# iliasam/STM32F4_SDR_GPS

Measured on AMD Instinct MI355X. Metric: acquisition hypotheses/sec (PRN x Doppler x phase), higher is better.
Workload: dtype u1 (MX-FP4 operands, exact f32 accumulation)

## Files before the change

### stm32f4_sdr_gps_amd/csrc/gpsx_mx_transposed.hpp

```cpp
#pragma once
#include <stdint.h>

constexpr int kGpsxMxtLocals = 64;
constexpr int kGpsxMxtKeyShift = 6;
constexpr int kGpsxKeyShift = 11;

constexpr int gpsx_mxt_q0_tile(int wave) { return 8 * (wave >> 1) + (wave & 1); }
constexpr int gpsx_mxt_row(int h, int r) { return (r & 3) + 8 * (r >> 2) + 4 * h; }
constexpr int gpsx_mxt_q(int wave, int h, int j, int r) { return 32 * (gpsx_mxt_q0_tile(wave) + 2 * j) + gpsx_mxt_row(h, r); }
constexpr int gpsx_mxt_local(int j, int r) { return 16 * j + r; }
constexpr uint32_t gpsx_mxt_code(int j, int r) { return (uint32_t)(kGpsxMxtLocals - 1 - gpsx_mxt_local(j, r)); }
constexpr uint32_t gpsx_mxt_local_key(uint32_t bits, int j, int r) { return (bits << kGpsxMxtKeyShift) | gpsx_mxt_code(j, r); }
constexpr int gpsx_mxt_q_of_local(int q_first, int local)
{
  return q_first + ((local & 48) << 2) + ((local & 12) << 1) + (local & 3);
}
constexpr uint32_t gpsx_mxt_global_key(uint32_t local_key, int q_first, int half)
{
  const int local = (int)((local_key & (kGpsxMxtLocals - 1)) ^ (kGpsxMxtLocals - 1));
  const int q = gpsx_mxt_q_of_local(q_first, local);
  return ((local_key >> kGpsxMxtKeyShift) << kGpsxKeyShift) | (uint32_t)(2047 - (2 * q + half));
}
constexpr int gpsx_mxt_group(int lane) { return (lane & 31) >> 3; }
```

### stm32f4_sdr_gps_amd/csrc/k_acq_mx.hip

```cpp
#include "gpsx_mx_parts.hpp"
#include "gpsx_mx_transposed.hpp"

namespace gpsx {

__global__ void k_build_mx_tables(const u32 *__restrict__ chipbits, int n_slots, u32 *__restrict__ mx_a, u32 *__restrict__ mx_t)
{
  const int n_sets = (n_slots + 31) / 32;
  const int idx = blockIdx.x * blockDim.x + threadIdx.x;
  const int per_set = 16 * 2 * 32 * 4 + 1032;
  if (idx >= n_sets * per_set)
    return;
  const int set = idx / per_set, r = idx - set * per_set;
  if (r < 16 * 2 * 32 * 4) {
    const int dw = r & 3, p = (r >> 2) & 31, h = (r >> 7) & 1, kappa = r >> 8;
    const int slot = 32 * set + p;
    const u32 word = slot < n_slots ? chipbits[(size_t)slot * 32 + 2 * kappa + h] : 0u;
    mx_a[(size_t)set * (16 * 2 * 32 * 4) + r] = spread8((word >> (8 * dw)) & 0xFFu) << 1;
  } else {
    const int c = r - 16 * 2 * 32 * 4 - 1;
    u32 w = 0;
    if (c >= 0 && c < kChips)
      for (int p = 0; p < 32; p++) {
        const int slot = 32 * set + p;
        if (slot < n_slots)
          w |= ((chipbits[(size_t)slot * 32 + (c >> 5)] >> (c & 31)) & 1u) << p;
      }
    mx_t[(size_t)set * 1032 + (c + 1)] = w;
  }
}

void launch_build_mx_tables(hipStream_t s, const uint32_t *d_chipbits, int n_slots, uint32_t *d_mx_a, uint32_t *d_mx_t)
{
  const int n_sets = (n_slots + 31) / 32;
  const int n = n_sets * (16 * 2 * 32 * 4 + 1032);
  hipLaunchKernelGGL(k_build_mx_tables, dim3((n + 255) / 256), dim3(256), 0, s, d_chipbits, n_slots, d_mx_a, d_mx_t);
}

namespace {

constexpr int kMxNoSet = -1;
constexpr int kPasses = 17;
constexpr int kPassesAnchor = 16;
constexpr int kAnchorDwords = 392;

__device__ __forceinline__ void mx_planes_half(MxSharedCore &sh, int t0_lo, int v, int lane)
{
  const int iq = v >> 1, t0_first = t0_lo + 4 * (v & 1);
  const int t0 = t0_first + (lane & 3), rot = lane >> 2;
#pragma unroll 1
  for (int it = 0; it < 2; it++) {
    const int w = rot + 16 * it;
    const u32 *src = &sh.d[iq][16 * w];
    u32 bits = 0;
#pragma unroll
    for (int k = 0; k < 16; k++) {
      const int kk = (k + rot) & 15;
      const u32 sk = src[kk];
      bits |= ((sk >> t0) & 1u) << (2 * kk);
      bits |= ((sk >> (16 + t0)) & 1u) << (2 * kk + 1);
    }
    sh.plane[iq][t0][w] = bits;
  }
  __builtin_amdgcn_fence(__ATOMIC_ACQ_REL, "wavefront");
  asm volatile("s_waitcnt lgkmcnt(0)" ::: "memory");
#pragma unroll 1
  for (int m = lane; m < 4 * (kPlaneWordsMx - 32); m += 64) {
    const int r = m / (kPlaneWordsMx - 32), w = 32 + m % (kPlaneWordsMx - 32);
    u32 *pl = sh.plane[iq][t0_first + r];
    pl[w] = mx_plane_ext_word(pl, w);
  }
}

__device__ __forceinline__ void mx_anchor_build(MxSharedCore &sh, u32 *dst, int tid)
{
  const int iq = tid >> 8, j = tid & 255;
  const u32 *dd = sh.d[iq];
  u64 bits = 0;
#pragma unroll
  for (int e = 0; e < 8; e++) {
    const int pos = 16 * wrap1023(8 * j + e);
    const u32 sum = pop16(__builtin_amdgcn_alignbit(dd[(pos >> 5) + 1], dd[pos >> 5], (u32)(pos & 31)));
    bits |= (u64)gpsx_anchor_code((int)sum) << (6 * e);
  }
  const u32 lo = (u32)bits, hi = (u32)(bits >> 32);
  const u32 lo_pair = dpp<0xB1>(lo, lo);
  u32 *d3 = dst + iq * kAnchorDwords + 3 * (j >> 1);
  if (j & 1) {
    d3[2] = (lo >> 16) | (hi << 16);
  } else {
    d3[0] = lo;
    d3[1] = hi | (lo_pair << 16);
  }
}

struct AnchorRaw {
  u32 d[7];
};
__device__ __forceinline__ AnchorRaw mx_anchor_raw(lds_cu32 *w, int dw)
{
  AnchorRaw r;
#pragma unroll
  for (int i = 0; i < 7; i++)
    r.d[i] = w[dw + i];
  return r;
}
__device__ __forceinline__ v8i mx_anchor_frag(const AnchorRaw &r, u32 shift)
{
  v8i f = {0, 0, 0, 0, 0, 0, 0, 0};
#pragma unroll
  for (int i = 0; i < 6; i++)
    f[i] = (int)__builtin_amdgcn_alignbit(r.d[i + 1], r.d[i], shift);
  return f;
}
template <int S, int NT>
__device__ __forceinline__ void mx_anchor_step(lds_cu32 *wi, lds_cu32 *wq, const v4i *ca, v4i (&a)[16], v8i &fi, v8i &fq,
                                               v16f (&acc)[2][NT], u32 shift)
{
  constexpr int kSteps = 16 + NT - 1;
  constexpr bool more = S + 1 < kSteps;
  AnchorRaw ri, rq;
  if constexpr (more) {
    ri = mx_anchor_raw(wi, 12 * (S + 1));
    rq = mx_anchor_raw(wq, 12 * (S + 1));
    if constexpr (S + 1 < 16)
      a[S + 1] = ca[(S + 1) * 64];
  }
  constexpr int j_lo = S - 15 > 0 ? S - 15 : 0, j_hi = S < NT - 1 ? S : NT - 1;
#pragma unroll
  for (int j = j_lo; j <= j_hi; j++) {
    acc[0][j] = __builtin_amdgcn_mfma_scale_f32_32x32x64_f8f6f4(fi, widen(a[S - j]), acc[0][j], 3, 4, 0, kScaleTwo, 0, kScaleA);
    acc[1][j] = __builtin_amdgcn_mfma_scale_f32_32x32x64_f8f6f4(fq, widen(a[S - j]), acc[1][j], 3, 4, 0, kScaleTwo, 0, kScaleA);
  }
  if constexpr (more) {
    __builtin_amdgcn_sched_group_barrier(0x100, S + 1 < 16 ? 9 : 8, 0);
    __builtin_amdgcn_sched_group_barrier(0x008, 2 * (j_hi - j_lo + 1), 0);
  }
  __builtin_amdgcn_sched_barrier(0);
  if constexpr (more) {
    fi = mx_anchor_frag(ri, shift);
    fq = mx_anchor_frag(rq, shift);
    __builtin_amdgcn_sched_barrier(0);
    mx_anchor_step<S + 1, NT>(wi, wq, ca, a, fi, fq, acc, shift);
  }
}
template <int NT>
__device__ __forceinline__ void mx_anchor_pass(const MxSharedCore &sh, const u32 *anchor, int lane, int q0_tile, v16f (&acc)[2][NT])
{
  const int n = lane & 31, h = lane >> 5;
  const u32 shift = (u32)(6 * n) & 31u;
  lds_cu32 *wi = lds_opaque(anchor + 6 * (q0_tile + h) + ((6 * n) >> 5));
  lds_cu32 *wq = lds_opaque(anchor + kAnchorDwords + 6 * (q0_tile + h) + ((6 * n) >> 5));
  const v4i *ca = &sh.chips_a[0][h][n];
  v4i a[16];
  v8i fi = mx_anchor_frag(mx_anchor_raw(wi, 0), shift), fq = mx_anchor_frag(mx_anchor_raw(wq, 0), shift);
  a[0] = ca[0];
  mx_anchor_step<0, NT>(wi, wq, ca, a, fi, fq, acc, shift);
}

__device__ __forceinline__ void mx_vector_build_direct(MxShared &sh, int which, int t0s, u32 *e8_dst, int tid)
{
  const int iq = tid >> 8, j = tid & 255;
  const u32 *dd = sh.d[iq];
  u32 w2[2] = {0, 0};
#pragma unroll
  for (int e = 0; e < 16; e++) {
    const int k = wrap1023(8 * j + e);
    const int pos = 16 * k + t0s;
    const u32 sum = pop16(__builtin_amdgcn_alignbit(dd[(pos >> 5) + 1], dd[pos >> 5], (u32)(pos & 31)));
    const u32 code = which == 0 ? (0xFEC0u >> (4u * (sum & 3u))) & 0xFu : (0xEDCA0u >> (4u * (sum >> 2))) & 0xFu;
    w2[e >> 3] |= code << (4 * (e & 7));
  }
  u32 *dst = e8_dst + (iq * 8) * kCopyDwords + j;
#pragma unroll
  for (int c = 0; c < 8; c++)
    dst[c * kCopyDwords] = c ? __builtin_amdgcn_alignbit(w2[1], w2[0], 4u * (u32)c) : w2[0];
}

__device__ __forceinline__ void mx_direct_terms(const MxShared &sh, int lane, int q0_tile, v16f (&acc)[2][kMxTiles], int t0s,
                                                int win_start, int win_stop)
{
  const int n = lane & 31, h = lane >> 5;
  const int b = t0s & 7, half = t0s >> 3;
  const u32 low = (1u << b) - 1u, high = (0xFFFFu << b) & 0xFFFFu;
  const float fh = (float)half;
  const u32 f22 = sh.chip_t[1022 + 1] >> (4 * h), f21 = sh.chip_t[1021 + 1] >> (4 * h);
  float popw[2], beta[2];
#pragma unroll
  for (int s = 0; s < 2; s++) {
    const int pw = (int)__popc(sh.d[s][0] & 0xFFu);
    popw[s] = (float)pw;
    beta[s] = (float)(16 - b - 2 * pw);
  }
#pragma unroll
  for (int j = 0; j < kMxTiles; j++) {
    const int q = 32 * (q0_tile + 2 * j) + n;
    const bool exists = q < kChips;
    const int qc = exists ? q : 0;
    const int o = 2 * qc + half;
    const float tq = (qc > 0) ? fh : 0.0f;
    float k0[2], k21[2], k22[2], kb[2];
#pragma unroll
    for (int s = 0; s < 2; s++) {
      const int fa = 2 * (int)__popc(lds_byte(sh.d[s], o) & low) - b;
      int fp = 0, gl = 0, gh = 0;
      if (qc > 0 || half == 0) {
        const int o2 = o >= 2 ? o : 2;
        const u32 prev = lds_byte(sh.d[s], o2 - 2) | (lds_byte(sh.d[s], o2 - 1) << 8);
        fp = (int)__popc(prev);
        gl = b - 2 * (int)__popc(prev & low);
        gh = 16 - b - 2 * (int)__popc(prev & high);
      }
      k0[s] = -(fh * popw[s] + tq * (float)fp) * kAccScale;
      k21[s] = -tq * (float)gl * kAccScale;
      k22[s] = ((float)fa - tq * (float)gh) * kAccScale;
      kb[s] = -fh * beta[s] * kAccScale;
    }
    const float ka = -fh * (float)b * kAccScale;
    if (half) {
      const bool in0 = exists && 2 * q >= win_start && 2 * q < win_stop;
      const bool in1 = exists && 2 * q + 1 >= win_start && 2 * q + 1 < win_stop;
      if (in0 != in1) {
        k0[0] += in1 ? -kOutside : kOutside;
        k0[1] += in1 ? -kOutside : kOutside;
      }
    }
    const u32 w1 = sh.chip_t[(exists ? kChips - 1 - q : 0) + 1] >> (4 * h);
    const u32 w0 = sh.chip_t[(exists ? kChips - 2 - q : -1) + 1] >> (4 * h);
#pragma unroll
    for (int r = 0; r < 16; r++) {
      const int pb = (r & 3) + 8 * (r >> 2);
      const float c22 = (float)((f22 >> pb) & 1u), c21 = (float)((f21 >> pb) & 1u);
      const float ca = (float)((w0 >> pb) & 1u), cb = (float)((w1 >> pb) & 1u);
      acc[0][j][r] += k0[0] + ca * ka + cb * kb[0] + c21 * k21[0] + c22 * k22[0];
      acc[1][j][r] += k0[1] + ca * ka + cb * kb[1] + c21 * k21[1] + c22 * k22[1];
    }
  }
}

template <bool S16>
struct SumRecT {
  u32 w[S16 ? 2 : 3];
};
template <bool S16>
__device__ __forceinline__ void sums_unpack(const SumRecT<S16> &r, u32 (&s)[4])
{
  if constexpr (S16) {
    s[0] = r.w[0] & 0xFFFFu;
    s[1] = r.w[0] >> 16;
    s[2] = r.w[1] & 0xFFFFu;
    s[3] = r.w[1] >> 16;
  } else {
    s[0] = r.w[0] & 0xFFFFFFu;
    s[1] = __builtin_amdgcn_alignbit(r.w[1], r.w[0], 24u) & 0xFFFFFFu;
    s[2] = __builtin_amdgcn_alignbit(r.w[2], r.w[1], 16u) & 0xFFFFFFu;
    s[3] = r.w[2] >> 8;
  }
}
template <bool S16>
__device__ __forceinline__ SumRecT<S16> sums_pack(const u32 (&s)[4])
{
  SumRecT<S16> r;
  if constexpr (S16) {
    r.w[0] = __builtin_amdgcn_perm(s[1], s[0], 0x05040100u);
    r.w[1] = __builtin_amdgcn_perm(s[3], s[2], 0x05040100u);
  } else {
    r.w[0] = s[0] | (s[1] << 24);
    r.w[1] = (s[1] >> 8) | (s[2] << 16);
    r.w[2] = (s[2] >> 16) | (s[3] << 8);
  }
  return r;
}

typedef unsigned short us2 __attribute__((ext_vector_type(2)));
__device__ __forceinline__ u32 pk_add_sat_u16(u32 a, u32 b)
{
  return __builtin_bit_cast(u32, __builtin_elementwise_add_sat(__builtin_bit_cast(us2, a), __builtin_bit_cast(us2, b)));
}

template <bool S16>
struct alignas(8) RecPairT {
  SumRecT<S16> a, b;
};
template <int FIRST, int COUNT, bool S16>
__device__ __forceinline__ void mx_prefetch_sums(const u32 *__restrict__ energy, const u32 *__restrict__ zero_recs, int lane,
                                                 int t0, bool ms_first, SumRecT<S16> (&pre)[16])
{
  static_assert(FIRST % 2 == 0 && COUNT % 2 == 0, "records move in pairs");
  if constexpr (S16) {
    const SumRecT<S16> *e2 = ms_first ? reinterpret_cast<const SumRecT<S16> *>(zero_recs) + (size_t)lane * 2
                                      : reinterpret_cast<const SumRecT<S16> *>(energy) + (size_t)(t0 * kMxTiles) * 256 + (size_t)lane * 2;
#pragma unroll
    for (int i = FIRST; i < FIRST + COUNT; i += 2) {
      const RecPairT<S16> rp = *reinterpret_cast<const RecPairT<S16> *>(&e2[(size_t)(i >> 2) * 256 + (size_t)((i & 3) >> 1) * 128]);
      pre[i] = rp.a;
      pre[i + 1] = rp.b;
    }
    return;
  }
  const SumRecT<S16> *e4 = ms_first ? reinterpret_cast<const SumRecT<S16> *>(zero_recs) + (size_t)lane * 4
                                    : reinterpret_cast<const SumRecT<S16> *>(energy) + ((size_t)(t0 * kMxTiles) * 64 + lane) * 4;
#pragma unroll
  for (int i = FIRST; i < FIRST + COUNT; i += 2) {
    const RecPairT<S16> rp = *reinterpret_cast<const RecPairT<S16> *>(&e4[(size_t)(i >> 2) * 256 + (i & 3)]);
    pre[i] = rp.a;
    pre[i + 1] = rp.b;
  }
}

template <bool MULTI, bool SEARCH, bool S16>
__device__ __forceinline__ void mx_epilogue(MxShared &sh, int lane, int q0_tile, int t0, const v16f (&acc)[2][kMxTiles],
                                            u32 group_mask, u32 *__restrict__ energy, const u32 *__restrict__ zero_recs,
                                            SumRecT<S16> (&pre)[MULTI ? 16 : 1], bool ms_first, u32 &witness)
{
  typedef SumRecT<S16> SumRec;
  constexpr bool ms_last = SEARCH;
  const int n = lane & 31, h = lane >> 5;
  const int b = t0 & 7, half = t0 >> 3;
  constexpr bool DIRECT = MULTI;
  u32 *slot = SEARCH ? &sh.part[b][4 * h][0][n] : nullptr;
  u32 best[SEARCH && !DIRECT ? 16 : 1], total[SEARCH && !DIRECT ? 16 : 1];
#pragma unroll
  for (int r = 0; r < (SEARCH && !DIRECT ? 16 : 1); r++) {
    best[r] = 0;
    total[r] = 0;
  }
  SumRec *e4 = reinterpret_cast<SumRec *>(energy) + ((size_t)(t0 * kMxTiles) * 64 + lane) * 4;
  mx_round_toward_zero();
#pragma unroll
  for (int j = 0; j < kMxTiles; j++) {
    const int q = 32 * (q0_tile + 2 * j) + n;
    const u32 key_lo = (u32)(2047 - (2 * q + half));
    if constexpr (MULTI) {
      if (j == 0)
        mx_prefetch_sums<8, 8, S16>(energy, zero_recs, lane, t0, ms_first, pre);
    }
    constexpr int GS = MULTI ? 4 : 8;
    SumRec held{};
#pragma unroll
    for (int r0 = 0; r0 < 16; r0 += GS) {
      u32 prev[GS];
#pragma unroll
      for (int i = 0; i < GS; i++)
        prev[i] = 0;
      if (MULTI && !(S16 && !SEARCH)) {
#pragma unroll
        for (int g = 0; g < GS / 4; g++) {
          u32 p4[4];
          sums_unpack<S16>(pre[MULTI ? j * 4 + r0 / 4 + g : 0], p4);
#pragma unroll
          for (int i = 0; i < 4; i++) {
            prev[4 * g + i] = p4[i];
            if constexpr (S16)
              witness = max(witness, p4[i]);
          }
        }
      }
      SumRec *e_rec = e4 + (size_t)j * 256 + r0 / 4;
      u32 out[GS];
      float ev[GS];
      u32 e_max = 0;
#pragma unroll
      for (int i = 0; i < GS; i++) {
        ev[i] = clip_square_sum(acc[0][j][r0 + i], acc[1][j][r0 + i]);
        e_max = max(e_max, __float_as_uint(ev[i]));
      }
      const bool small = __builtin_amdgcn_ballot_w64(e_max >= 0x3C800000u ) == 0;
      u32 mag[GS];
      constexpr bool PACKED = MULTI && S16 && !SEARCH;
      if (small) {
#pragma unroll
        for (int i = 0; i < GS; i++)
          mag[i] = PACKED ? root_bits_small(ev[i]) : (u32)(int)(__builtin_amdgcn_sqrtf(ev[i]) * kRootGuard);
      } else {
        float ci[GS], cq[GS];
#pragma unroll
        for (int i = 0; i < GS; i++) {
          ci[i] = acc[0][j][r0 + i];
          cq[i] = acc[1][j][r0 + i];
        }
        mx_roots_exact<GS>(ci, cq, mag);
      }
      if constexpr (PACKED) {
        const SumRec &pr = pre[j * 4 + r0 / 4];
        SumRec nr;
        nr.w[0] = pk_add_sat_u16(pr.w[0], __builtin_amdgcn_perm(mag[1], mag[0], 0x05040100u));
        nr.w[1] = pk_add_sat_u16(pr.w[1], __builtin_amdgcn_perm(mag[3], mag[2], 0x05040100u));
        if ((r0 / 4) & 1) {
          RecPairT<S16> both;
          both.a = held;
          both.b = nr;
          SumRec *e_pair = reinterpret_cast<SumRec *>(energy) + (size_t)(t0 * kMxTiles + j) * 256 + (size_t)(r0 / 8) * 128 + (size_t)lane * 2;
          *reinterpret_cast<RecPairT<S16> *>(e_pair) = both;
        } else {
          held = nr;
        }
        __builtin_amdgcn_sched_barrier(0);
        continue;
      }
#pragma unroll
      for (int i = 0; i < GS; i++) {
        const int r = r0 + i;
        u32 val = mag[i];
        if (MULTI)
          val += prev[i];
        out[i] = val;
        if (SEARCH && DIRECT) {
          const int p_off = ((r & 3) + 8 * (r >> 2)) * 64;
          atomicMax(slot + p_off, (val << 11) | key_lo);
          atomicAdd(slot + p_off + 32, val);
        } else if (SEARCH) {
          const u32 key = (val << 11) | key_lo;
          best[DIRECT ? 0 : r] = key > best[DIRECT ? 0 : r] ? key : best[DIRECT ? 0 : r];
          total[DIRECT ? 0 : r] += val;
        }
      }
      if (MULTI && !ms_last) {
#pragma unroll
        for (int g = 0; g < GS / 4; g++) {
          const u32 o4[4] = {out[4 * g], out[4 * g + 1], out[4 * g + 2], out[4 * g + 3]};
          e_rec[g] = sums_pack<S16>(o4);
        }
      }
      if (SEARCH && !DIRECT) {
#pragma unroll
        for (int i = 0; i < GS; i++)
          asm volatile("" : "+v"(best[DIRECT ? 0 : r0 + i]), "+v"(total[DIRECT ? 0 : r0 + i]));
      }
      __builtin_amdgcn_sched_barrier(0);
    }
  }
  mx_round_to_nearest();
  if (SEARCH && !DIRECT) {
#pragma unroll
    for (int r = 0; r < 16; r++) {
      const int p_off = ((r & 3) + 8 * (r >> 2)) * 64;
      atomicMax(slot + p_off, best[DIRECT ? 0 : r]);
      atomicAdd(slot + p_off + 32, total[DIRECT ? 0 : r]);
    }
  }
}

__device__ __forceinline__ void mx_epilogue_store(int lane, int q0_tile, int t0, const v16f (&acc)[2][kMxTiles], u32 group_mask,
                                                  uint16_t *__restrict__ plane0, size_t prn_stride, int slot0, int n_prn)
{
  const int n = lane & 31, h = lane >> 5;
#pragma unroll
  for (int j = 0; j < kMxTiles; j++) {
    const int q = 32 * (q0_tile + 2 * j) + n;
    uint16_t *v = plane0 + (size_t)t0 * 1024 + (size_t)(q & 3) * 256 + (size_t)(q >> 2);
#pragma unroll
    for (int g = 0; g < 4; g++) {
#pragma unroll
      for (int rr = 0; rr < 4; rr++) {
        const int r = 4 * g + rr;
        const int p = (r & 3) + 8 * (r >> 2) + 4 * h;
        const u32 val = mag8_f32(acc[0][j][r], acc[1][j][r]);
        if (((group_mask >> g) & 1u) && slot0 + p < n_prn)
          v[(size_t)p * prn_stride] = (uint16_t)val;
      }
      __builtin_amdgcn_sched_barrier(0);
    }
  }
}

constexpr int kHsStride = 1026;
struct MxSingleShared {
  MxSharedCore mx;
  MxFold fold;
  alignas(16) u32 part[8][2][2][32];
  alignas(16) float2 hs[2][kHsStride];
};

struct MxtWindow {
  int lo0, hi0, lo1, hi1;
};
__device__ __forceinline__ MxtWindow mxt_window(int win_start, int win_stop)
{
  MxtWindow w;
  w.lo0 = (win_start + 1) >> 1;
  w.hi0 = min(kChips, (win_stop + 1) >> 1);
  w.lo1 = win_start >> 1;
  w.hi1 = min(kChips, win_stop >> 1);
  return w;
}
__device__ __forceinline__ bool mxt_wave_whole(int q0_tile, int win_start, int win_stop)
{
  const MxtWindow w = mxt_window(win_start, win_stop);
  const int q_lo = 32 * q0_tile, q_hi = 32 * (q0_tile + 2 * (kMxTiles - 1)) + 31;
  return q_lo >= w.lo0 && q_hi < w.hi1;
}

__device__ __forceinline__ void mxt_init_acc(const u32 *ones, int lane, int q0_tile, v16f (&acc)[2][kMxTiles], int win_start,
                                             int win_stop, int pass_bias)
{
  const float base_i = (float)((int)ones[0] + 8192 - kHalf - pass_bias) * kAccScale,
              base_q = (float)((int)ones[1] + 8192 - kHalf - pass_bias) * kAccScale;
  if (mxt_wave_whole(q0_tile, win_start, win_stop)) {
#pragma unroll
    for (int j = 0; j < kMxTiles; j++)
#pragma unroll
      for (int r = 0; r < 16; r++) {
        acc[0][j][r] = base_i;
        acc[1][j][r] = base_q;
      }
  } else {
    const MxtWindow w = mxt_window(win_start, win_stop);
    const int h = lane >> 5;
    const u32 span = (u32)max(w.hi0 - w.lo0, 0);
#pragma unroll
    for (int j = 0; j < kMxTiles; j++)
#pragma unroll
      for (int r = 0; r < 16; r++) {
        const int q = 32 * (q0_tile + 2 * j) + gpsx_mxt_row(h, r);
        const bool in_win = (u32)(q - w.lo0) < span;
        acc[0][j][r] = in_win ? base_i : base_i + kOutside;
        acc[1][j][r] = in_win ? base_q : base_q + kOutside;
      }
  }
}

__device__ __forceinline__ void mxt_half_switch_build(const MxSharedCore &sh, float2 (*hs)[kHsStride], int t, int n)
{
  const int popw[2] = {(int)__popc(sh.d[0][0] & 0xFFu), (int)__popc(sh.d[1][0] & 0xFFu)};
#pragma unroll 1
  for (int m = t; m < 512; m += n) {
    float row[2][2][2];
#pragma unroll
    for (int s = 0; s < 2; s++) {
      const u32 w = sh.d[s][m], before = sh.d[s][m > 0 ? m - 1 : 0] >> 24;
#pragma unroll
      for (int k = 0; k < 2; k++) {
        const u32 cur = (w >> (16 * k)) & 0xFFu;
        int fa = -(2 * (int)__popc(cur & 0x7Fu) - 7);
        int fk = -popw[s];
        if (2 * m + k > 0) {
          const u32 prev = (k ? (w >> 8) & 0xFFu : before) | (cur << 8);
          fk -= (int)__popc(prev);
          fa -= 16 - 2 * (int)__popc(prev);
        }
        row[0][k][s] = (float)fk * kAccScale;
        row[1][k][s] = (float)(fk + fa) * kAccScale;
      }
    }
#pragma unroll
    for (int c = 0; c < 2; c++)
      *reinterpret_cast<float4 *>(&hs[c][2 * m]) = make_float4(row[c][0][0], row[c][0][1], row[c][1][0], row[c][1][1]);
  }
}

__device__ __forceinline__ void mxt_half_switch(const MxSharedCore &sh, const float2 (*hs)[kHsStride], int lane, int q0_tile,
                                                v16f (&acc)[2][kMxTiles], int win_start, int win_stop)
{
  asm volatile("" : "+v"(lane));
  const int prn = lane & 31, h = lane >> 5;
  const u32 wrap_i = (sh.d[0][0] & 0xFFu) << 8, wrap_q = (sh.d[1][0] & 0xFFu) << 8;
  const float nbeta_i = -(float)(16 - 2 * (int)__popc(wrap_i)) * kAccScale, nbeta_q = -(float)(16 - 2 * (int)__popc(wrap_q)) * kAccScale;
  const int q4_first = 32 * q0_tile + 4 * h, q4_last = q4_first + 64 * (kMxTiles - 1) + 24;
  const float2 *tab = &hs[(sh.chip_t[1022 + 1] >> prn) & 1u][q4_first];
  const u32 *cw = &sh.chip_t[kChips - 3 - q4_last];
#pragma unroll
  for (int j = 0; j < kMxTiles; j++) {
#pragma unroll
    for (int g = 0; g < 4; g++) {
      const int dq = 64 * j + 8 * g;
      const float4 t01 = *reinterpret_cast<const float4 *>(&tab[dq]), t23 = *reinterpret_cast<const float4 *>(&tab[dq + 2]);
      const uint4 w = *reinterpret_cast<const uint4 *>(&cw[64 * (kMxTiles - 1) + 24 - dq]);
      const float ti[4] = {t01.x, t01.z, t23.x, t23.z}, tq[4] = {t01.y, t01.w, t23.y, t23.w};
      const u32 wi[4] = {w.w, w.z, w.y, w.x};
#pragma unroll
      for (int i = 0; i < 4; i++) {
        const float c1 = (float)((wi[i] >> prn) & 1u);
        acc[0][j][4 * g + i] += __builtin_fmaf(c1, nbeta_i, ti[i]);
        acc[1][j][4 * g + i] += __builtin_fmaf(c1, nbeta_q, tq[i]);
      }
    }
  }
  if (!mxt_wave_whole(q0_tile, win_start, win_stop)) {
    const MxtWindow w = mxt_window(win_start, win_stop);
    const bool any = win_start < win_stop;
    const int q_in = any && w.lo1 != w.lo0 ? w.lo1 : -1, q_out = any && w.hi1 != w.hi0 ? w.hi1 : -1;
#pragma unroll
    for (int j = 0; j < kMxTiles; j++) {
      const int tile = q0_tile + 2 * j;
      if ((q_in >> 5) != tile && (q_out >> 5) != tile)
        continue;
#pragma unroll
      for (int r = 0; r < 16; r++) {
        const int q = 32 * tile + gpsx_mxt_row(h, r);
        const float edge = (q == q_in ? -kOutside : 0.0f) + (q == q_out ? kOutside : 0.0f);
        acc[0][j][r] += edge;
        acc[1][j][r] += edge;
      }
    }
  }
}

__device__ __forceinline__ void mxt_epilogue(u32 *part, int lane, int q0_tile, int t0, const v16f (&acc)[2][kMxTiles])
{
  const int b = t0 & 7, half = t0 >> 3;
  u32 best[4], total[4];
#pragma unroll
  for (int c = 0; c < 4; c++) {
    best[c] = 0;
    total[c] = c ? 0u : 0u - (u32)kGpsxMxtLocals * kRootBias;
  }
  mx_round_toward_zero();
#pragma unroll
  for (int jp = 0; jp < kMxTiles; jp += 2) {
#pragma unroll
    for (int r0 = 0; r0 < 16; r0 += 4) {
      float ev[8];
      u32 e_max = 0;
#pragma unroll
      for (int i = 0; i < 8; i++) {
        ev[i] = clip_square_sum(acc[0][jp + (i >> 2)][r0 + (i & 3)], acc[1][jp + (i >> 2)][r0 + (i & 3)]);
        e_max = max(e_max, __float_as_uint(ev[i]));
      }
      const bool small = __builtin_amdgcn_ballot_w64(e_max >= 0x3C800000u ) == 0;
      u32 bits[8];
      if (__builtin_expect(small, 1)) {
#pragma unroll
        for (int i = 0; i < 8; i++)
          bits[i] = root_bits_small(ev[i]);
      } else {
        float ci[8], cq[8];
#pragma unroll
        for (int i = 0; i < 8; i++) {
          ci[i] = acc[0][jp + (i >> 2)][r0 + (i & 3)];
          cq[i] = acc[1][jp + (i >> 2)][r0 + (i & 3)];
        }
        mx_roots_exact<8>(ci, cq, bits);
#pragma unroll
        for (int i = 0; i < 8; i++)
          bits[i] += kRootBias;
      }
#pragma unroll
      for (int rr = 0; rr < 4; rr++) {
        const u32 k0 = gpsx_mxt_local_key(bits[rr], jp, r0 + rr), k1 = gpsx_mxt_local_key(bits[4 + rr], jp + 1, r0 + rr);
        best[rr] = max(max(best[rr], k0), k1);
        total[rr] = total[rr] + bits[rr] + bits[4 + rr];
      }
#pragma unroll
      for (int rr = 0; rr < 4; rr++)
        asm volatile("" : "+v"(best[rr]), "+v"(total[rr]));
      __builtin_amdgcn_sched_barrier(0);
    }
  }
  mx_round_to_nearest();
  const u32 key = gpsx_mxt_global_key(max(max(best[0], best[1]), max(best[2], best[3])), 32 * q0_tile + 4 * (lane >> 5), half);
  u32 *slot = part + (2 * b) * 64 + lane;
  atomicMax(slot, key);
  atomicAdd(slot + 64, total[0] + total[1] + total[2] + total[3]);
}
__device__ __forceinline__ void mx_fill_fold_lut(MxFold &fold, int t)
{
  if (t < 64) {
    const int late = t >> 5, z = t & 31;
    v4i e;
#pragma unroll
    for (int i = 0; i < 4; i++)
      e[i] = (int)(gpsx_fold_pair(late != 0, 2, (z >> i) & 1, (z >> (i + 1)) & 1) << kGpsxFoldShift);
    fold.lut[late][z] = e;
  }
}

__device__ __forceinline__ void mx_single(MxSingleShared &shs, const AcqParams &prm, int cluster_lo,
                                          const uint8_t *__restrict__ if_blocks, const u32 *__restrict__ mx_a,
                                          const u32 *__restrict__ mx_t, gpsx_peak_t *__restrict__ peaks)
{
  MxSharedCore &sh = shs.mx;
  MxFold &fold = shs.fold;
  u32 *part = &shs.part[0][0][0][0];
  const int tid = threadIdx.x;
  const int lane = tid & 63, wave = __builtin_amdgcn_readfirstlane(tid >> 6);
  const int role = wave >> 2;
  const int q0_tile = 8 * (wave >> 1) + (wave & 1);

  const int n_sets = (prm.n_groups + 3) / 4;
  const MxCluster c = mx_decode_cluster(cluster_lo + (int)blockIdx.x, n_sets, prm.n_dopp);
  const int set = c.set, sd = c.sd, dopp = c.dopp, search = c.search;
  u32 group_mask = 0;
#pragma unroll
  for (int g = 0; g < 4; g++) {
    const int group = 4 * set + g;
    const int unit = sd * prm.n_groups + group;
    if (group < prm.n_groups && unit >= prm.unit_lo && unit < prm.unit_hi)
      group_mask |= 1u << g;
  }
  group_mask = (u32)__builtin_amdgcn_readfirstlane((int)group_mask);
  if (group_mask == 0)
    return;
  const u32 step_word = mx_step_word(dopp, prm.if_hz, prm.dopp_min_hz, prm.dopp_step_hz);

  if (set != kMxNoSet) {
    mx_load_tables(sh, mx_a, mx_t, set, tid);
  }
  if (tid < (int)(sizeof(shs.part) / sizeof(uint4)))
    reinterpret_cast<uint4 *>(part)[tid] = make_uint4(0, 0, 0, 0);
  const size_t block_bytes = prm.if_format == GPSX_IF_2BIT_SM ? GPSX_BYTES_PER_MS_2BIT : kBytes;
  const uint8_t *block0 = if_blocks + (size_t)(search * prm.search_stride_blocks) * block_bytes;
  mx_load_block(sh, block0, prm.if_format, tid);

  __syncthreads();
  const int n_pass = kPassesAnchor;
#pragma unroll 1
  for (int once = 0; once < 1; once++) {
    mx_wipe_stream<true>(sh, step_word, tid, lane);
    __syncthreads();
    mx_anchor_build(sh, &sh.e8[0][0][0][0], tid);

    v16f acc[2][kMxTiles];
    if (role == 0)
      mxt_init_acc(sh.ones, lane, q0_tile, acc, prm.win_start, prm.win_stop, kGpsxAnchorPassBias);

    auto opaque = [](int v) {
      asm volatile("" : "+v"(v));
      return v;
    };
    __syncthreads();
    if (role) {
      mx_planes_half(sh, 0, wave & 3, opaque(lane));
      mx_fill_tables(sh, opaque(tid) & 255, 256);
      mx_fill_fold_lut(fold, opaque(tid) & 255);
      mx_planes_half(sh, 8, wave & 3, opaque(lane));
      mxt_half_switch_build(sh, shs.hs, opaque(tid) & 255, 256);
      mxt_init_acc(sh.ones, opaque(lane), q0_tile, acc, prm.win_start, prm.win_stop, kGpsxAnchorPassBias);
    }
    mx_anchor_pass(sh, &sh.e8[0][0][0][0], lane, q0_tile, acc);
    if (!role)
      mxt_epilogue(part, lane, q0_tile, 0, acc);
    __syncthreads();
    mx_vector_build<true>(sh, 2, opaque(tid), &fold);
#pragma unroll 1
    for (int hs = 2; hs <= 2 * n_pass; hs++) {
      if ((hs & 1) == 0) {
        __syncthreads();
        const int p_vec = (hs >> 1) + 1;
        if (p_vec < n_pass)
          mx_vector_build<true>(sh, p_vec + 1, tid, &fold);
      }
      const int x = hs - role;
      const bool active = x >= 0 && x < 2 * n_pass;
      const int p = (x >> 1) + 1;
      if (active && (x & 1) == 0) {
        mx_pass<true, kMxTiles, kScaleA, true>(sh, p & 1, lane, q0_tile, acc, p == 1 ? kScaleEight : kScaleOne, v4i{0, 0, 0, 0},
                                               p >= 2 && p != 9, &fold.pair[p & 1][0][0]);
        if (p == 9)
          mxt_half_switch(sh, shs.hs, lane, q0_tile, acc, prm.win_start, prm.win_stop);
      }
      if (active && (x & 1) && p >= 1)
        mxt_epilogue(part, lane, q0_tile, p - 1, acc);
    }
  }
  __syncthreads();
  {
    const int which = tid >> 8, p = (tid >> 3) & 31, b = tid & 7;
    const int slot = 32 * set + p;
    const u32 v0 = shs.part[b][which][0][p], v1 = shs.part[b][which][1][p];
    const u32 k = v0 > v1 ? v0 : v1, t = v0 + v1;
    if (((group_mask >> (p >> 3)) & 1u) && slot < prm.n_prn && b < prm.n_bits) {
      const size_t idx = ((size_t)(search * prm.n_prn + slot) * prm.n_dopp + dopp) * prm.n_bits + b;
      uint2 *pk = reinterpret_cast<uint2 *>(&peaks[idx]);
      if (which == 0) {
        const u32 max_val = k >> 11;
        pk[0] = make_uint2(max_val, max_val ? 2047u - (k & 2047u) : 0u);
      } else {
        pk[1] = make_uint2(t, t / (2u * kChips));
      }
    }
    if (prm.keys && which == 0) {
      unsigned long long key = 0;
      if (b < prm.n_bits) {
        const u32 max_val = k >> 11, phase = max_val ? 2047u - (k & 2047u) : 0u;
        key = ((unsigned long long)max_val << 14) | (unsigned long long)(16383u - (8u * phase + (u32)b));
      }
      key = mx_max8_u64(key);
      if (b == 0 && ((group_mask >> (p >> 3)) & 1u) && slot < prm.n_prn)
        prm.keys[(size_t)(search * prm.n_prn + slot) * prm.n_dopp + dopp] = (int64_t)key;
    }
  }
}

template <int MODE>
__device__ __forceinline__ void mx_unit(MxShared &sh, const AcqParams &prm, int cluster_lo,
                                        const uint8_t *__restrict__ if_blocks, const u32 *__restrict__ mx_a,
                                        const u32 *__restrict__ mx_t, gpsx_peak_t *__restrict__ peaks, u32 *__restrict__ energy,
                                        u32 *__restrict__ flags)
{
  constexpr bool MULTI = MODE == kMxWalk || MODE == kMxWalk16, STORE = MODE == kMxStore, S16 = MODE == kMxWalk16;
  constexpr bool SPLIT = MODE == kMxSplit;
  typedef SumRecT<S16> SumRec;
  const int wg = (int)blockIdx.x;
  if constexpr (MODE == kMxWalk) {
    if (flags && flags[wg] == 0)
      return;
  }
  const int tid = threadIdx.x;
  const int lane = tid & 63, wave = __builtin_amdgcn_readfirstlane(tid >> 6);
  const int role = wave >> 2;
  const int q0_tile = 8 * (wave >> 1) + (wave & 1);

  const int n_sets = (prm.n_groups + 3) / 4;
  const int ms_store = STORE ? wg % prm.n_ms : 0;
  const int n_seg = SPLIT ? prm.split_segs : 1;
  const int seg = SPLIT ? wg % n_seg : 0;
  const MxCluster c = mx_decode_cluster(cluster_lo + (STORE ? wg / prm.n_ms : SPLIT ? wg / n_seg : wg), n_sets, prm.n_dopp);
  const int set = c.set, sd = c.sd, dopp = c.dopp, search = c.search;
  u32 group_mask = 0;
#pragma unroll
  for (int g = 0; g < 4; g++) {
    const int group = 4 * set + g;
    const int unit = sd * prm.n_groups + group;
    if (group < prm.n_groups && unit >= prm.unit_lo && unit < prm.unit_hi)
      group_mask |= 1u << g;
  }
  group_mask = (u32)__builtin_amdgcn_readfirstlane((int)group_mask);
  if (group_mask == 0)
    return;
  const u32 step_word = mx_step_word(dopp, prm.if_hz, prm.dopp_min_hz, prm.dopp_step_hz);

  if (set != kMxNoSet) {
    mx_load_tables(sh, mx_a, mx_t, set, tid);
    mx_fill_tables(sh, tid);
  }
  for (int i = tid; i < 8 * 32 * 2 * 32 / 4; i += kMxThreads)
    reinterpret_cast<uint4 *>(&sh.part[0][0][0][0])[i] = make_uint4(0, 0, 0, 0);
  const size_t block_bytes = prm.if_format == GPSX_IF_2BIT_SM ? GPSX_BYTES_PER_MS_2BIT : kBytes;
  const uint8_t *block0 = if_blocks + (size_t)(search * prm.search_stride_blocks + (STORE ? wg % prm.n_ms : 0)) * block_bytes;
  mx_load_block(sh, block0, prm.if_format, tid);

  __syncthreads();
  const v4i a_corr = v4i{(int)(((sh.chip_t[(lane >> 5 ? 1021 : 1022) + 1] >> (lane & 31)) & 1u) << 1), 0, 0, 0};
  u32 kq[kMxTiles];
#pragma unroll
  for (int j = 0; j < kMxTiles; j++) {
    kq[j] = (u32)(2047 - 2 * (32 * (q0_tile + 2 * j) + (lane & 31)));
    if constexpr (!MULTI && !STORE)
      asm volatile("" : "+v"(kq[j]));
  }
  u32 *e_wave = MULTI ? energy + ((size_t)wg * 8 + wave) * (16 * kMxTiles * 4 * 64 * (S16 ? 2 : 3)) : nullptr;
  const u32 *zero_recs = MULTI ? flags - kMxZeroRecBytes / sizeof(u32) : nullptr;
  u32 witness = 0;
  const int n_ms = MULTI ? prm.n_ms : 1;
  const int t0s = SPLIT ? seg * (16 / n_seg) : 0;
  const int n_pass = SPLIT ? 16 / n_seg + 1 : kPasses;
  const int pbase = t0s;
#pragma unroll 1
  for (int ms = 0; ms < n_ms; ms++) {
    const bool ms_first = ms == 0, ms_last = ms == n_ms - 1;
    int tid_p = tid, lane_p = lane;
    if constexpr (MULTI)
      asm volatile("" : "+v"(tid_p), "+v"(lane_p));
    if (ms > 0) {
      __syncthreads();
      mx_load_block(sh, block0 + (size_t)ms * block_bytes, prm.if_format, tid_p);
      __syncthreads();
    }
    if (SPLIT && seg) {
      mx_wipe_block(sh, step_word, tid_p, lane_p);
      mx_vector_build_direct(sh, 0, t0s, &sh.e8[0][0][0][0], tid);
      mx_vector_build_direct(sh, 1, t0s, &sh.e8[1][0][0][0], tid);
      for (int i = tid; i < 2 * 2 * 2 * 128; i += kMxThreads)
        (&sh.corr[0][0][0][0])[i] = 0;
    } else {
      mx_wipe_block(sh, step_word, tid_p, lane_p);
      __syncthreads();
      mx_vector_phase1(sh, 0, 0, tid_p);
      __syncthreads();
      mx_vector_phase2(sh, 0, tid_p);
      __syncthreads();
      mx_vector_phase1(sh, 1, 1, tid_p);
      __syncthreads();
      mx_vector_phase2(sh, 1, tid_p);
    }

    v16f acc[2][kMxTiles];
    mx_init_acc(sh.ones, lane_p, q0_tile, acc, prm.win_start, prm.win_stop);
    SumRec pre[MULTI ? 16 : 1];

#pragma unroll 1
    for (int hs = 0; hs <= 2 * n_pass; hs++) {
      if ((hs & 1) == 0)
        __syncthreads();
      constexpr bool kBuildBehindEpilogue = MULTI;
      if (!kBuildBehindEpilogue && (hs & 1) == 0) {
        const int p_vec = (hs >> 1) + 1;
        if (p_vec >= 2 && p_vec < n_pass) {
          int tid_v = tid;
          if constexpr (MULTI)
            asm volatile("" : "+v"(tid_v));
          mx_vector_build(sh, pbase + p_vec, tid_v);
        }
      }
      int lane_s = lane;
      if constexpr (MULTI)
        asm volatile("" : "+v"(lane_s));
      const int x = hs - role;
      const bool active = x >= 0 && x < 2 * n_pass;
      const int p = x >> 1;
      if (active && (x & 1) == 0) {
        if constexpr (MULTI) {
          if (p >= 1)
            mx_prefetch_sums<0, 8, S16>(e_wave, zero_recs, lane_s, p - 1, ms_first, pre);
        }
        mx_pass<!MULTI>(sh, p & 1, lane, q0_tile, acc, p == 1 ? kScaleEight : kScaleOne, a_corr, p >= 2 && (SPLIT || p != 9));
        if constexpr (SPLIT) {
          if (p == 1 && seg) {
            int lane_d = lane;
            asm volatile("" : "+v"(lane_d));
            mx_direct_terms(sh, lane_d, q0_tile, acc, t0s, prm.win_start, prm.win_stop);
          }
        } else {
          if (p == 9)
            mx_half_switch(sh, lane_s, q0_tile, acc, prm.win_start, prm.win_stop);
        }
      }
      if (STORE) {
        if (active && (x & 1) && p >= 1) {
          uint16_t *plane0 = reinterpret_cast<uint16_t *>(energy) +
                             ((size_t)((search * prm.n_ms + ms_store) * prm.n_prn + 32 * set) * prm.n_dopp + dopp) * (16 * 1024);
          mx_epilogue_store(lane, q0_tile, p - 1, acc, group_mask, plane0, (size_t)prm.n_dopp * (16 * 1024), 32 * set, prm.n_prn);
        }
      } else if (active && (x & 1) && p >= 1) {
        if (!MULTI)
          mx_epilogue_single(sh, lane, kq, t0s + p - 1, acc);
        else if (!ms_last)
          mx_epilogue<MULTI, false, S16>(sh, lane_s, q0_tile, p - 1, acc, group_mask, e_wave, zero_recs, pre, ms_first, witness);
        else
          mx_epilogue<MULTI, true, S16>(sh, lane_s, q0_tile, p - 1, acc, group_mask, e_wave, zero_recs, pre, ms_first, witness);
      }
      if (kBuildBehindEpilogue && (x & 1) != 0) {
        const int p_vec = (hs >> 1) + 1;
        if (p_vec >= 2 && p_vec < n_pass) {
          int tid_v = tid;
          if constexpr (MULTI)
            asm volatile("" : "+v"(tid_v));
          mx_vector_build(sh, pbase + p_vec, tid_v);
        }
      }
    }
  }
  if (STORE)
    return;
  if constexpr (S16) {
    if (tid == 0)
      sh.ones[0] = 0;
    __syncthreads();
    if (__builtin_amdgcn_ballot_w64(witness >= 0xFFFFu) != 0 && lane == 0)
      atomicOr(&sh.ones[0], 1u);
  }
  __syncthreads();
  if constexpr (S16) {
    if (tid == 0)
      flags[wg] = sh.ones[0];
    if (sh.ones[0])
      return;
  }
  {
    const int which = tid >> 8, p = (tid >> 3) & 31, b = tid & 7;
    const int slot = 32 * set + p;
    const u32 *row = sh.part[b][p][which];
    u32 vals[32];
#pragma unroll
    for (int l = 0; l < 32; l++)
      vals[l] = row[(l + tid) & 31];
    u32 k = 0, t = 0;
#pragma unroll
    for (int l = 0; l < 32; l++) {
      k = vals[l] > k ? vals[l] : k;
      t += vals[l];
    }
    if (((group_mask >> (p >> 3)) & 1u) && slot < prm.n_prn && b < prm.n_bits) {
      const size_t idx = ((size_t)(search * prm.n_prn + slot) * prm.n_dopp + dopp) * prm.n_bits + b;
      uint2 *pk = reinterpret_cast<uint2 *>(&peaks[idx]);
      if constexpr (SPLIT) {
        const size_t n_planes = (size_t)prm.n_planes;
        if (which == 0)
          atomicMax(&energy[idx], k);
        else
          atomicAdd(&energy[n_planes + idx], t);
      } else if (which == 0) {
        const u32 max_val = k >> 11;
        pk[0] = make_uint2(max_val, max_val ? 2047u - (k & 2047u) : 0u);
      } else {
        pk[1] = make_uint2(t, t / (2u * kChips));
      }
    }
    if constexpr (!SPLIT) {
      if (prm.keys && which == 0) {
        unsigned long long key = 0;
        if (b < prm.n_bits) {
          const u32 max_val = k >> 11, phase = max_val ? 2047u - (k & 2047u) : 0u;
          key = ((unsigned long long)max_val << 14) | (unsigned long long)(16383u - (8u * phase + (u32)b));
        }
        key = mx_max8_u64(key);
        if (b == 0 && ((group_mask >> (p >> 3)) & 1u) && slot < prm.n_prn)
          prm.keys[(size_t)(search * prm.n_prn + slot) * prm.n_dopp + dopp] = (int64_t)key;
      }
    }
  }
}

}

template <int MODE>
__global__ __launch_bounds__(kMxThreads, 1) void k_acq_mx(GPSX_K_ACQ_MX_PARAMS)
{
  if constexpr (MODE == kMxSingle) {
    __shared__ MxSingleShared sh;
    mx_single(sh, prm, cluster_lo, if_blocks, mx_a, mx_t, peaks);
  } else {
    __shared__ MxShared sh;
    mx_unit<MODE>(sh, prm, cluster_lo, if_blocks, mx_a, mx_t, peaks, energy, flags);
  }
}

void launch_acq_mx(hipStream_t s, const AcqPlan &p, const AcqParams &prm, const uint8_t *d_if, const uint32_t *d_mx_a,
                   const uint32_t *d_mx_t, uint32_t *d_planes, uint32_t *d_energy)
{
  if (p.c_hi <= p.c_lo)
    return;
  const dim3 grid((unsigned)p.grid), block(kMxThreads);
  gpsx_peak_t *d_peaks = prm.peaks;
  switch (p.form) {
  case AcqForm::kMxStore:
    hipLaunchKernelGGL(k_acq_mx<kMxStore>, grid, block, 0, s, prm, p.c_lo, d_if, d_mx_a, d_mx_t, d_peaks, d_energy, (u32 *)nullptr);
    launch_acq_vals_search(s, prm, reinterpret_cast<const uint16_t *>(d_energy), d_peaks, p.n_peaks);
    break;
  case AcqForm::kMxWalk: {
    u32 *d_flags = d_energy + acq_mx_energy_bytes(p.grid) / sizeof(u32) - p.grid;
    (void)hipMemsetAsync(d_flags - kMxZeroRecBytes / sizeof(u32), 0, kMxZeroRecBytes, s);
    hipLaunchKernelGGL(k_acq_mx<kMxWalk16>, grid, block, 0, s, prm, p.c_lo, d_if, d_mx_a, d_mx_t, d_peaks, d_energy, d_flags);
    if (p.walk24)
      hipLaunchKernelGGL(k_acq_mx<kMxWalk>, grid, block, 0, s, prm, p.c_lo, d_if, d_mx_a, d_mx_t, d_peaks, d_energy, d_flags);
    break;
  }
  case AcqForm::kMxByte:
    launch_acq_mx_byte(s, (unsigned)p.grid, prm, p.c_lo, d_if, d_mx_a, d_mx_t);
    break;
  case AcqForm::kMxSplit:
    hipLaunchKernelGGL(k_acq_mx<kMxSplit>, grid, block, 0, s, prm, p.c_lo, d_if, d_mx_a, d_mx_t, d_peaks, d_planes, (u32 *)nullptr);
    launch_acq_finalize(s, d_planes, d_planes + p.n_peaks, p.n_peaks, d_peaks, prm.keys);
    break;
  default:
    hipLaunchKernelGGL(k_acq_mx<kMxSingle>, grid, block, 0, s, prm, p.c_lo, d_if, d_mx_a, d_mx_t, d_peaks, (u32 *)nullptr,
                       (u32 *)nullptr);
    if (p.form != AcqForm::kMxTail)
      break;
    hipLaunchKernelGGL(k_acq_mx<kMxSplit>, dim3((unsigned)p.grid_tail), block, 0, s, prm, p.c_tail, d_if, d_mx_a, d_mx_t, d_peaks,
                       d_planes, (u32 *)nullptr);
    launch_acq_finalize_from(s, d_planes, d_planes + p.n_peaks, p.first_peak, p.n_peaks, d_peaks, prm.n_prn, prm.n_dopp,
                             prm.n_bits, (prm.n_groups + 3) / 4, p.c_tail, prm.keys);
  }
}

}
```

Before: 1509 billion.

## Add speculative fast sqrt epilogue with hot-state fallback to exact roots

The epilogue now first runs a fast path that computes roots with a hardware sqrt plus an FMA bias trick, keeping chains in explicit phases. It falls back to the original exact or ballot path only when the winning key reaches a trust radius, and it carries a per-wave 'hot' flag so later passes go straight to the careful path once magnitudes get large. The aim is to remove the per-group ballot and branch in the common low-magnitude case and to schedule the ALU chains better. The cost is duplicated code and more registers, and correctness depends on the radius thresholds bounding the approximation error.

```diff
diff --git a/stm32f4_sdr_gps_amd/csrc/gpsx_mx_transposed.hpp b/stm32f4_sdr_gps_amd/csrc/gpsx_mx_transposed.hpp
--- a/stm32f4_sdr_gps_amd/csrc/gpsx_mx_transposed.hpp
+++ b/stm32f4_sdr_gps_amd/csrc/gpsx_mx_transposed.hpp
@@ -21,4 +21,10 @@
   const int q = gpsx_mxt_q_of_local(q_first, local);
   return ((local_key >> kGpsxMxtKeyShift) << kGpsxKeyShift) | (uint32_t)(2047 - (2 * q + half));
 }
+constexpr uint32_t kGpsxMxtRootBias = 0x4B000000u;
+constexpr int kGpsxMxtTrustRadius = 1024;
+constexpr int kGpsxMxtHotRadius = 768;
+constexpr uint32_t gpsx_mxt_limit_key(int radius) { return (kGpsxMxtRootBias + (uint32_t)radius) << kGpsxMxtKeyShift; }
+constexpr uint32_t gpsx_mxt_trust_limit_key() { return gpsx_mxt_limit_key(kGpsxMxtTrustRadius); }
+constexpr uint32_t gpsx_mxt_hot_limit_key() { return gpsx_mxt_limit_key(kGpsxMxtHotRadius); }
 constexpr int gpsx_mxt_group(int lane) { return (lane & 31) >> 3; }
diff --git a/stm32f4_sdr_gps_amd/csrc/k_acq_mx.hip b/stm32f4_sdr_gps_amd/csrc/k_acq_mx.hip
--- a/stm32f4_sdr_gps_amd/csrc/k_acq_mx.hip
+++ b/stm32f4_sdr_gps_amd/csrc/k_acq_mx.hip
@@ -595,49 +595,84 @@
   }
 }
 
-__device__ __forceinline__ void mxt_epilogue(u32 *part, int lane, int q0_tile, int t0, const v16f (&acc)[2][kMxTiles])
-{
-  const int b = t0 & 7, half = t0 >> 3;
+static_assert(kGpsxMxtRootBias == kRootBias, "gpsx_mx_transposed.hpp's limit keys carry the small path's bias");
+static_assert(kGpsxMxtHotRadius <= kGpsxMxtTrustRadius, "mxt_epilogue tests the limit only where the predictor's radius is reached");
+template <typename T>
+__device__ __forceinline__ void mxt_phase(T (&v)[8])
+{
+  asm volatile("" : "+v"(v[0]), "+v"(v[1]), "+v"(v[2]), "+v"(v[3]), "+v"(v[4]), "+v"(v[5]), "+v"(v[6]), "+v"(v[7]));
+  __builtin_amdgcn_sched_barrier(0);
+}
+template <bool TRUST>
+__device__ __forceinline__ u32 mxt_chains(const v16f (&acc)[2][kMxTiles], u32 &sum)
+{
   u32 best[4], total[4];
 #pragma unroll
   for (int c = 0; c < 4; c++) {
     best[c] = 0;
     total[c] = c ? 0u : 0u - (u32)kGpsxMxtLocals * kRootBias;
   }
-  mx_round_toward_zero();
 #pragma unroll
   for (int jp = 0; jp < kMxTiles; jp += 2) {
 #pragma unroll
     for (int r0 = 0; r0 < 16; r0 += 4) {
-      float ev[8];
-      u32 e_max = 0;
-#pragma unroll
-      for (int i = 0; i < 8; i++) {
-        ev[i] = clip_square_sum(acc[0][jp + (i >> 2)][r0 + (i & 3)], acc[1][jp + (i >> 2)][r0 + (i & 3)]);
-        e_max = max(e_max, __float_as_uint(ev[i]));
-      }
-      const bool small = __builtin_amdgcn_ballot_w64(e_max >= 0x3C800000u ) == 0;
       u32 bits[8];
-      if (__builtin_expect(small, 1)) {
+      if constexpr (TRUST) {
+        float si[8], sq[8], ev[8], rt[8];
+#pragma unroll
+        for (int i = 0; i < 8; i++) {
+          si[i] = mx_clip_square(acc[0][jp + (i >> 2)][r0 + (i & 3)]);
+          sq[i] = mx_clip_square(acc[1][jp + (i >> 2)][r0 + (i & 3)]);
+        }
+        mxt_phase(si);
+        mxt_phase(sq);
 #pragma unroll
         for (int i = 0; i < 8; i++)
-          bits[i] = root_bits_small(ev[i]);
+          ev[i] = si[i] + sq[i];
+        mxt_phase(ev);
+#pragma unroll
+        for (int i = 0; i < 8; i++)
+          rt[i] = __builtin_amdgcn_sqrtf(ev[i]);
+        mxt_phase(rt);
+#pragma unroll
+        for (int i = 0; i < 8; i++)
+          bits[i] = __float_as_uint(__builtin_fmaf(rt[i], kRootGuard, 8388608.0f));
+        mxt_phase(bits);
       } else {
-        float ci[8], cq[8];
+        float ev[8];
+        u32 e_max = 0;
 #pragma unroll
         for (int i = 0; i < 8; i++) {
-          ci[i] = acc[0][jp + (i >> 2)][r0 + (i & 3)];
-          cq[i] = acc[1][jp + (i >> 2)][r0 + (i & 3)];
-        }
-        mx_roots_exact<8>(ci, cq, bits);
-#pragma unroll
-        for (int i = 0; i < 8; i++)
-          bits[i] += kRootBias;
-      }
+          ev[i] = clip_square_sum(acc[0][jp + (i >> 2)][r0 + (i & 3)], acc[1][jp + (i >> 2)][r0 + (i & 3)]);
+          e_max = max(e_max, __float_as_uint(ev[i]));
+        }
+        const bool small = __builtin_amdgcn_ballot_w64(e_max >= 0x3C800000u ) == 0;
+        if (__builtin_expect(small, 1)) {
+#pragma unroll
+          for (int i = 0; i < 8; i++)
+            bits[i] = root_bits_small(ev[i]);
+        } else {
+          float ci[8], cq[8];
+#pragma unroll
+          for (int i = 0; i < 8; i++) {
+            ci[i] = acc[0][jp + (i >> 2)][r0 + (i & 3)];
+            cq[i] = acc[1][jp + (i >> 2)][r0 + (i & 3)];
+          }
+          mx_roots_exact<8>(ci, cq, bits);
+#pragma unroll
+          for (int i = 0; i < 8; i++)
+            bits[i] += kRootBias;
+        }
+      }
+      u32 key[8];
+#pragma unroll
+      for (int i = 0; i < 8; i++)
+        key[i] = gpsx_mxt_local_key(bits[i], jp + (i >> 2), r0 + (i & 3));
+      if constexpr (TRUST)
+        mxt_phase(key);
 #pragma unroll
       for (int rr = 0; rr < 4; rr++) {
-        const u32 k0 = gpsx_mxt_local_key(bits[rr], jp, r0 + rr), k1 = gpsx_mxt_local_key(bits[4 + rr], jp + 1, r0 + rr);
-        best[rr] = max(max(best[rr], k0), k1);
+        best[rr] = max(max(best[rr], key[rr]), key[4 + rr]);
         total[rr] = total[rr] + bits[rr] + bits[4 + rr];
       }
 #pragma unroll
@@ -646,11 +681,34 @@
       __builtin_amdgcn_sched_barrier(0);
     }
   }
+  sum = total[0] + total[1] + total[2] + total[3];
+  return max(max(best[0], best[1]), max(best[2], best[3]));
+}
+__device__ __forceinline__ void mxt_epilogue(u32 *part, int lane, int q0_tile, int t0, v16f (&acc)[2][kMxTiles], bool &hot)
+{
+  const int b = t0 & 7, half = t0 >> 3;
+  u32 winner = 0, sum = 0;
+  bool careful = hot;
+  mx_round_toward_zero();
+  if (!careful) {
+    winner = mxt_chains<true>(acc, sum);
+    hot = __builtin_amdgcn_ballot_w64(winner >= gpsx_mxt_hot_limit_key()) != 0;
+    careful = hot && __builtin_amdgcn_ballot_w64(winner >= gpsx_mxt_trust_limit_key()) != 0;
+  }
+  if (careful) {
+#pragma unroll
+    for (int s = 0; s < 2; s++)
+#pragma unroll
+      for (int j = 0; j < kMxTiles; j++)
+        asm volatile("" : "+v"(acc[s][j]));
+    winner = mxt_chains<false>(acc, sum);
+    hot = __builtin_amdgcn_ballot_w64(winner >= gpsx_mxt_hot_limit_key()) != 0;
+  }
   mx_round_to_nearest();
-  const u32 key = gpsx_mxt_global_key(max(max(best[0], best[1]), max(best[2], best[3])), 32 * q0_tile + 4 * (lane >> 5), half);
+  const u32 key = gpsx_mxt_global_key(winner, 32 * q0_tile + 4 * (lane >> 5), half);
   u32 *slot = part + (2 * b) * 64 + lane;
   atomicMax(slot, key);
-  atomicAdd(slot + 64, total[0] + total[1] + total[2] + total[3]);
+  atomicAdd(slot + 64, sum);
 }
 __device__ __forceinline__ void mx_fill_fold_lut(MxFold &fold, int t)
 {
@@ -727,8 +785,9 @@
       mxt_init_acc(sh.ones, opaque(lane), q0_tile, acc, prm.win_start, prm.win_stop, kGpsxAnchorPassBias);
     }
     mx_anchor_pass(sh, &sh.e8[0][0][0][0], lane, q0_tile, acc);
+    bool hot = false;
     if (!role)
-      mxt_epilogue(part, lane, q0_tile, 0, acc);
+      mxt_epilogue(part, lane, q0_tile, 0, acc, hot);
     __syncthreads();
     mx_vector_build<true>(sh, 2, opaque(tid), &fold);
 #pragma unroll 1
@@ -749,7 +808,7 @@
           mxt_half_switch(sh, shs.hs, lane, q0_tile, acc, prm.win_start, prm.win_stop);
       }
       if (active && (x & 1) && p >= 1)
-        mxt_epilogue(part, lane, q0_tile, p - 1, acc);
+        mxt_epilogue(part, lane, q0_tile, p - 1, acc, hot);
     }
   }
   __syncthreads();
```

New measurement: 1535 billion (median of 6 runs). 1.7% higher.
